# informalsystems/ed25519-consensus

Hardware: AMD Instinct MI355X
Metric: Ed25519 batch-verified signatures/sec (whole node) at 2^20 sigs (higher is better)
Workload: dtype u32/u64 integer (GF(2^255-19), radix 2^29 limbs); 1 GPU; configs[2]: 2^20 votes/GPU from 150 validators, 120-byte msgs; sigs_per_gpu=1048576, validators=150, msg_len=120, inflight=6, keycache=False, prehashed=False, batches_per_launch=1, multi_union_first=False, parallelism=single

## Files before the change

ed25519-consensus_amd/csrc/edc_api.hip:

```cpp
#include <stdlib.h>
#include <string.h>
#include <string>
#include <random>
#include <algorithm>
#include <chrono>
#include <condition_variable>
#include <initializer_list>
#include <mutex>
#include <thread>
#include <unordered_map>
#include <vector>
#include <errno.h>
#include <sys/random.h>
#include <hip/hip_ext.h>
#include "edc.h"
#include "edc_common.h"
#include "edc_launch.h"
#include "vfy_fold.h"
#include "vfy_cached.h"
#include "tmpl.h"
#include "commits.h"
#include "quorum.h"
#include "valset.h"
#include "vhist.h"
// ... 456 lines not shown
    else dens[w] = nf / half;
    total += split ? ns + 2 * nf : (w < P.nwin_short ? ns + nf : nf);
  }
  double target = ctx->bin_entries ? (double)ctx->bin_entries : (total / 1024.0 > 4096.0 ? total / 1024.0 : 4096.0);
  for (;;) {
    for (uint32_t w = 0; w < P.nwin; ++w) P.nsub[w] = (uint8_t)floor_pow2(dens[w] / target);
    plan_layout(P);
    if (P.bins_per_range <= MSM_MAX_BINS) break;
    target *= 2;
  }
  note_plan(ctx, P, target, per_sig, split, few, false);
  return P;
}

static MsmTerms batch_terms(const MsmPlan& P, const Slot& s, uint32_t n, bool split, uint32_t skip = 0) {
  return MsmTerms{n - skip, 0, 0, 0, P.sum_ranges ? P.nranges : 1u, s.scal, nullptr, nullptr, nullptr, split ? 1u : 0u,
                  0u, skip};
}

static bool choose_split(const edc_ctx* ctx) {
  return ctx->kc_m && ctx->bcomb && ctx->key_split == 0 && ctx->last_uncached == 0;
}

static int ensure_n(edc_ctx* ctx, size_t n) {
  CK(grow_group(ctx->cap_n, n, item_cap, sync_of(ctx->st()), [&](size_t cap) {
    return alloc_all(sized(ctx->vtab, verify_single_scratch_words(cap)), sized(ctx->vk, cap * 32), sized(ctx->sig, cap * 64),
                     sized(ctx->zexp, cap * 16), sized(ctx->off, cap + 1), sized(ctx->kbuf, cap * 8), sized(ctx->verdicts, cap));
  }));
  return 0;
}

// ... 132 lines not shown
  x = (x ^ (x >> 30)) * 0xBF58476D1CE4E5B9ull;
  x = (x ^ (x >> 27)) * 0x94D049BB133111EBull;
  return x ^ (x >> 31);
}

static bool choose_per_sig(const edc_ctx* ctx, size_t n) {
  return ctx->key_grouping == 2 || (ctx->key_grouping == 0 && n >= 4096 && ctx->have_key_ratio &&
                                    ctx->last_key_ratio > 0.5 && ctx->ungrouped_run < 7);
}

static uint32_t key_lanes(const edc_ctx* ctx, size_t n, bool per_sig) {
  if (per_sig || !ctx->have_key_ratio) return (uint32_t)n;
  const double m2 = 2.0 * ctx->last_key_ratio * (double)n;
  const size_t lanes = m2 < 4096.0 ? 4096 : (size_t)m2 + 64;
  return (uint32_t)(lanes < n ? lanes : n);
}

static void slot_begin(Slot& s, const uint32_t* kin, uint32_t nmulti, bool timed, bool per_sig, uint32_t n) {
  s.kin = kin;
  s.nmulti = nmulti;
  s.timed = timed;
  s.per_sig = per_sig;
  s.n_batch = n;
}
static size_t batch_entry_room(const MsmPlan& P, size_t n, bool split) {
  return split ? msm_entry_capacity(P, 2 + 3 * n, 0) : msm_entry_capacity(P, n, n + 1);
}
static uint32_t batch_term_count(uint32_t n, bool split) { return split ? 2 + 3 * n : 1 + 2 * n; }

struct KeyTable {
// ... 49 lines not shown
  mark(PH_KEYS);
  const bool clear_counts = with_bin && EDC_RUN(8);
  launch_front(st, s, kt, N, d_vk, clear_counts ? s.msm.counts.get() : nullptr, clear_counts ? P->nbin() : 0u);
  const bool dual = EDC_DUAL_STREAM && s.st2 && !s.timed;
  mark(PH_CHALLENGE);
  if (!d_k && EDC_RUN(2)) launch_challenge(st, N, d_vk, d_sig, in.msg, in.off, s.k);
  if (dual) {
    CK(hipEventRecord(s.ev_keys, st));
    CK(hipStreamWaitEvent(s.st2, s.ev_keys, 0));
    if (EDC_RUN(16))
      launch_decompress(s.st2, N, d_sig, d_vk, s.key_rep, per_sig, s.pts, s.itembad + s.cap_n, s.keybad, s.flags,
                        ctx->kc(), split, key_lanes(ctx, n, per_sig));
    CK(hipEventRecord(s.ev_dec, s.st2));
  }
  mark(PH_COEF);
  if (EDC_RUN(4)) launch_coef(st, N, d_sig, s.kin, d_z, seed, in.z_base, s.key_index, s.scal, s.key_acc, s.u_acc, s.itembad, s.flags,
              per_sig, s.coef_part, split);
  mark(PH_MSM_BIN);
  if (with_bin && EDC_RUN(8))
    launch_msm_bin(st, *P, batch_terms(*P, s, N, split), batch_term_count(N, split), s.msm, s.flags, true);
  if (with_bin && EDC_RUN(256)) launch_msm_sort(st, *P, s.msm);
  mark(PH_DECOMP);
  if (dual) CK(hipStreamWaitEvent(st, s.ev_dec, 0));
  else if (EDC_RUN(16))
    launch_decompress(st, N, d_sig, d_vk, s.key_rep, per_sig, s.pts, s.itembad + s.cap_n, s.keybad, s.flags, ctx->kc(),
                      split, key_lanes(ctx, n, per_sig));
  CK(hipGetLastError());
  return 0;
}

static int enqueue_batch(edc_ctx* ctx, Slot& s, size_t n, const BatchIn& in, bool latency = false) {
  if (n >= (1ull << 28)) { ctx->err = "batch too large for one call (max 2^28 items)"; return EDC_ERR_ARG; }
  int rc = ensure_slot(ctx, s, n);
  if (rc) return rc;
  const bool per_sig = choose_per_sig(ctx, n), split = choose_split(ctx);
// ... 5365 lines not shown
```

ed25519-consensus_amd/csrc/edc_common.h:

```cpp
#pragma once
#include <hip/hip_runtime.h>
#include <stdint.h>
#include "fe25519.h"
#include "ge25519.h"
#include "sc25519.h"
#include "sha512.h"
#include "chacha20.h"
#include "keycache.h"

namespace edc {

constexpr int NIELS_WORDS = 32;
constexpr int EXT_WORDS = 36;

__device__ __forceinline__ fe ld_fe(const uint32_t* p) {
  fe r;
#pragma unroll
  for (int i = 0; i < 9; ++i) r.v[i] = p[i];
  return r;
}
__device__ __forceinline__ void st_fe(uint32_t* p, const fe& a) {
#pragma unroll
  for (int i = 0; i < 9; ++i) p[i] = a.v[i];
}
// ... 40 lines not shown
constexpr int SLICE_BITS = 8;
constexpr int NSLICE = 1 << SLICE_BITS;
constexpr uint32_t MSM_MAX_BINS = 8192;

struct MsmPlan {
  uint32_t nwin, nwin_short;
  uint32_t nranges;
  uint32_t sum_ranges;
  uint32_t bins_per_range;
  uint16_t off[MSM_MAX_WIN];
  uint8_t bits[MSM_MAX_WIN];
  uint8_t nsub[MSM_MAX_WIN];
  uint16_t bin0[MSM_MAX_WIN];
  uint16_t nslice[MSM_MAX_WIN];
  __host__ __device__ uint32_t nbin() const { return nranges * bins_per_range; }
};

struct MsmTerms {
  uint32_t n, rsize, npoint, nx;
  uint32_t nparts;
  const uint32_t* scal;
  const uint32_t* xpt;
  const uint32_t* xrg;
  const uint32_t* xscal;
  uint32_t split;
  uint32_t dyn;
  uint32_t skip;
};

__device__ __forceinline__ int plan_digit(const uint32_t s[8], uint32_t off, uint32_t bits, int& carry,
                                          bool top_unsigned) {
  const uint32_t k = off >> 5, sh = off & 31;
  const uint64_t two = (uint64_t)s[k] | ((uint64_t)(k < 7 ? s[k + 1] : 0u) << 32);
  const uint32_t raw = ((uint32_t)(two >> sh) & ((1u << bits) - 1u)) + (uint32_t)carry;
  if (top_unsigned) { carry = 0; return (int)raw; }
  if (raw >= (1u << (bits - 1))) { carry = 1; return (int)raw - (int)(1u << bits); }
  carry = 0;
  return (int)raw;
}

constexpr int KEY_ACC_LIMBS = 12;

enum { FLAG_BAD = 0, FLAG_NKEYS = 1, FLAG_VERDICT = 2, FLAG_OVF = 3, FLAG_UNCACHED = 4, FLAG_KARG = 5, FLAG_COUNT = 8 };
constexpr int FLAG_ALLOC = 32, FLAG_STAMP0 = 16;
enum { BST_INIT, BST_COEF, BST_COUNT, BST_DECODE, BST_ACCUM, BST_REDUCE, BST_FINAL, BST_END, BST_N };
#ifdef EDC_BATCH_STAMPS
#define BATCH_STAMP(fl, k)                                                                          \
  do {                                                                                              \
    if (blockIdx.x == 0 && threadIdx.x == 0 && (fl))                                                \
      const_cast<int*>(fl)[FLAG_STAMP0 + (k)] = (int)__builtin_amdgcn_s_memrealtime();              \
  } while (0)
#else
#define BATCH_STAMP(fl, k) do { } while (0)
// ... 17 lines not shown
```

ed25519-consensus_amd/csrc/edc_launch.h:

```cpp
#pragma once
#include <hip/hip_runtime.h>
#include <stdint.h>
#include "keycache.h"
#include "edc_common.h"
#include "devbuf.h"

namespace edc {
void launch_challenge(hipStream_t st, uint32_t n, const uint8_t* vk, const uint8_t* sig,
                      const uint8_t* msg, const uint64_t* off, uint32_t* k);
void launch_decompress(hipStream_t st, uint32_t n, const uint8_t* sig, const uint8_t* vk, const uint32_t* key_rep,
                       bool per_sig, uint32_t* pts, uint8_t* itembad, uint8_t* keybad, int* flags,
                       const KeyCacheView& kc, bool split = false, uint32_t klanes = 0);
void launch_decompress_range(hipStream_t st, uint32_t n, uint32_t r0, uint32_t rcnt, uint32_t klanes, const uint8_t* sig,
                             const uint8_t* vk, const uint32_t* key_rep, bool per_sig, uint32_t* pts, uint8_t* itembad,
                             uint8_t* keybad, int* flags, const KeyCacheView& kc, bool split = false);
void launch_keys(hipStream_t st, uint32_t n, const uint8_t* vk, uint32_t* table, uint32_t tmask,
                 const uint32_t salt[2], bool force_overflow, uint32_t* slot_key, uint32_t* key_slot_of_sig,
                 uint32_t* key_rep, uint32_t* key_index, unsigned long long* key_acc, int* flags,
                 uint32_t kcap = 0xFFFFFFFFu);
void launch_keys_range(hipStream_t st, uint32_t n0, uint32_t m, const uint8_t* vk, uint32_t* table, uint32_t tmask,
                       const uint32_t salt[2], bool force_overflow, bool seed_pass, uint32_t* slot_key,
                       uint32_t* key_slot_of_sig, uint32_t* key_rep, uint32_t* key_index, unsigned long long* key_acc,
                       uint32_t* kpts, uint32_t* khi, uint8_t* keybad, int* flags, const KeyCacheView& kc);
void launch_verifier_begin(hipStream_t st, uint32_t n, int* flags, unsigned long long* key_acc,
                           unsigned long long* u_acc, uint8_t* d_out, uint32_t* counts, uint32_t nbin);
void launch_verifier_place_keys(hipStream_t st, uint32_t n, const uint8_t* vk, const uint32_t* kpts, const uint32_t* khi,
                                uint32_t* pts, uint8_t* keybad, int* flags, const KeyCacheView& kc, bool split);
void launch_z_range(hipStream_t st, const uint32_t seed[8], uint32_t a, uint32_t cnt, uint32_t* scal);
void launch_coef(hipStream_t st, uint32_t n, const uint8_t* sig, const uint32_t* k, const uint8_t* zexp,
                 const uint32_t seed[8], uint64_t zbase, const uint32_t* key_index, uint32_t* scal,
                 unsigned long long* key_acc, unsigned long long* u_acc, uint8_t* itembad, int* flags,
                 bool per_sig, uint32_t* coef_part, bool split = false);
void launch_coef_range(hipStream_t st, uint32_t n, uint32_t item0, uint32_t cnt, const uint8_t* sig, const uint32_t* k,
                       const uint8_t* zexp, const uint32_t seed[8], uint64_t zbase, const uint32_t* key_index,
                       uint32_t* scal, unsigned long long* key_acc, unsigned long long* u_acc, uint8_t* itembad,
                       int* flags, bool per_sig, uint32_t* coef_part, bool split = false);
void launch_coef_finish(hipStream_t st, uint32_t n, unsigned long long* key_acc, unsigned long long* u_acc,
                        uint32_t* scal, int* flags, bool per_sig, uint32_t* coef_part, bool split = false);
size_t coef_part_words(size_t cap_n);
void launch_range_coef(hipStream_t st, uint32_t n, uint32_t rsize, uint32_t nranges, uint32_t m, bool per_sig,
                       const uint8_t* sig, const uint32_t* k, const uint8_t* zexp, const uint32_t seed[8],
                       uint64_t zbase, const uint32_t* key_index, uint32_t* scal, unsigned long long* key_acc,
                       unsigned long long* u_acc, int* flags, uint32_t* xpt, uint32_t* xrg, uint32_t* xscal);
void launch_multi_coef(hipStream_t st, uint32_t n, uint32_t nr, uint32_t kstride, bool per_sig, const uint8_t* sig,
                       const uint32_t* k, const uint32_t seed[8], uint64_t zbase, const uint32_t* key_index,
                       uint32_t* scal, unsigned long long* key_acc, unsigned long long* u_acc, uint8_t* itembad,
                       int* flags, uint32_t* xpt, uint32_t* xrg, uint32_t* xscal);
// ... 114 lines not shown
void launch_header_bind(hipStream_t st, const HeaderSrc& src, const HeaderBind& rules, const uint8_t* roots, uint8_t* bad,
                        uint32_t* n_bad);
hipError_t msm_init_device();
struct MsmWs {
  uint32_t cap_bins = 0, cap_ranges = 0;
  size_t cap_entries = 0;
  devbuf::DevBuf<uint32_t> counts, offsets, cursor;
  devbuf::DevBuf<uint2> entries;
  devbuf::DevBuf<uint32_t> sorted;
  devbuf::DevBuf<uint32_t> slice_W, slice_T, win;
  devbuf::DevBuf<uint32_t> buckets;
  devbuf::DevBuf<uint32_t> heads;
  devbuf::DevBuf<uint32_t> bucket_end;
};
void launch_msm_bin(hipStream_t st, const MsmPlan& P, const MsmTerms& T, uint32_t max_terms, MsmWs& ws, const int* flags,
                    bool counts_zeroed = false);
void launch_msm_sort(hipStream_t st, const MsmPlan& P, MsmWs& ws);
void launch_msm_bucket(hipStream_t st, const MsmPlan& P, MsmWs& ws, const uint32_t* pts, int probe_skip = 0,
                       hipEvent_t acc_begin = nullptr, hipEvent_t acc_end = nullptr, bool latency = false,
                       int* stamp_flags = nullptr);
size_t msm_bucket_words(uint32_t nbin);
void launch_msm_tail(hipStream_t st, const MsmPlan& P, MsmWs& ws, int* flags, int want_compress, uint8_t* out,
                     uint8_t* hout = nullptr, const uint32_t* extra = nullptr);
void launch_point_accum(hipStream_t st, uint32_t* run, const uint8_t* blk);
void launch_msm_range_tail(hipStream_t st, const MsmPlan& P, MsmWs& ws, uint8_t* rverdict);
void launch_msm_multi_tail(hipStream_t st, const MsmPlan& P, MsmWs& ws, const int* flags, const uint8_t* rbad,
                           int want_compress, uint8_t* out, uint8_t* hout);
void launch_combine_records(hipStream_t st, uint32_t g, const uint8_t* recs, uint32_t stride, uint8_t* out);
void launch_combine(hipStream_t st, uint32_t g, const uint8_t* partials, int bad, int want_compress,
                    uint8_t* out);
void launch_copy_block(hipStream_t st, const uint8_t* src, uint8_t* dst);
// ... 21 lines not shown
```

ed25519-consensus_amd/csrc/edc_msm.hip:

```cpp
#include "edc_common.h"
#include "edc_launch.h"
#include "ge_quad.h"
#include "ge_row.h"

namespace edc {


__device__ __forceinline__ MsmTerms resolve_terms(MsmTerms T, const int* flags) {
  if (T.dyn & 1u) {
    const bool per_sig = (T.dyn & 2u) || flags[FLAG_OVF];
    const uint32_t nr = T.nx, m = per_sig ? 0u : (uint32_t)flags[FLAG_NKEYS];
    T.npoint = per_sig ? 2 * T.n : T.n;
    T.nx = nr * m + nr;
  }
  return T;
}

__device__ __forceinline__ uint32_t terms_count(const MsmTerms& T, const int* flags) {
  if (T.rsize) return T.npoint + T.nx;
  const uint32_t m = (uint32_t)flags[FLAG_NKEYS];
  return T.split ? msm_num_points_split(T.n, m) : msm_num_points(T.n, m);
}

__device__ __forceinline__ void term_get(const MsmTerms& T, uint32_t t, uint32_t& pt, uint32_t& rg, bool& shrt,
                                         uint32_t s[8]) {
  const uint32_t* src;
  if (!T.rsize) {
    pt = t ? t + T.skip : 0u;
    rg = T.nparts > 1 ? t % T.nparts : 0;
    shrt = T.split || (t >= 1 && t <= T.n);
    src = T.scal + (size_t)pt * 8;
  } else if (t < T.npoint) {
    pt = 1 + T.skip + t;
    rg = (t < T.n ? t : t - T.n) / T.rsize;
    shrt = t < T.n;
    src = T.scal + (size_t)pt * 8;
  } else {
    const uint32_t q = t - T.npoint;
    pt = T.xpt[q];
    rg = T.xrg[q];
    shrt = false;
    src = T.xscal + (size_t)q * 8;
  }
  const uint4* q4 = reinterpret_cast<const uint4*>(src);
  const uint4 a = q4[0], b = shrt ? make_uint4(0u, 0u, 0u, 0u) : q4[1];
  s[0] = a.x; s[1] = a.y; s[2] = a.z; s[3] = a.w; s[4] = b.x; s[5] = b.y; s[6] = b.z; s[7] = b.w;
}

template <typename F>
__device__ __forceinline__ void term_digits(const MsmPlan& P, uint32_t t, bool shrt, uint32_t rg, const uint32_t s[8],
                                            F&& f) {
  const uint32_t nw = shrt ? P.nwin_short : P.nwin;
  const uint32_t rbase = rg * P.bins_per_range;
  int carry = 0;
  for (uint32_t w = 0; w < nw; ++w) {
    const int d = plan_digit(s, P.off[w], P.bits[w], carry, w + 1 == nw);
    if (d) {
      const uint32_t b = (uint32_t)(d < 0 ? -d : d) - 1;
      const uint32_t ns = P.nsub[w];
      f(rbase + P.bin0[w] + (b >> SLICE_BITS) * ns + (t & (ns - 1)), b & (NSLICE - 1), d < 0);
    }
  }
}

__global__ void __launch_bounds__(256) k_msm_count(MsmPlan P, MsmTerms T, uint32_t per_block,
                                                   uint32_t* __restrict__ counts, const int* __restrict__ flags) {
  extern __shared__ uint32_t hist[];
  BATCH_STAMP(flags, BST_COUNT);
  const uint32_t nbin = P.nbin();
  for (uint32_t b = threadIdx.x; b < nbin; b += blockDim.x) hist[b] = 0;
  __syncthreads();
  T = resolve_terms(T, flags);
  const uint32_t cnt = terms_count(T, flags);
  const uint32_t t0 = blockIdx.x * per_block;
  for (uint32_t u = threadIdx.x; u < per_block; u += blockDim.x) {
    const uint32_t t = t0 + u;
    if (t >= cnt) break;
    uint32_t pt, rg, s[8];
    bool shrt;
    term_get(T, t, pt, rg, shrt, s);
    term_digits(P, t, shrt, rg, s, [&](uint32_t bin, uint32_t, bool) { atomicAdd(&hist[bin], 1u); });
  }
  __syncthreads();
  for (uint32_t b = threadIdx.x; b < nbin; b += blockDim.x)
    if (hist[b]) atomicAdd(&counts[b], hist[b]);
}

__global__ void __launch_bounds__(1024) k_msm_scan(uint32_t nbin, const uint32_t* __restrict__ counts,
                                                   uint32_t* __restrict__ offsets,
                                                   uint32_t* __restrict__ cursor) {
  __shared__ uint32_t part[1024];
  const uint32_t t = threadIdx.x;
  const uint32_t per = (nbin + 1023) / 1024;
  const uint32_t b0 = t * per, b1 = min(nbin, b0 + per);
  uint32_t s = 0;
  for (uint32_t b = b0; b < b1; ++b) s += counts[b];
  part[t] = s;
  __syncthreads();
  for (int d = 1; d < 1024; d <<= 1) {
    uint32_t v = t >= (uint32_t)d ? part[t - d] : 0;
    __syncthreads();
    part[t] += v;
    __syncthreads();
  }
  uint32_t run = part[t] - s;
  for (uint32_t b = b0; b < b1; ++b) {
    offsets[b] = run;
    cursor[b] = run;
    run += counts[b];
  }
}

struct ScatterBlocks {
  uint32_t grid_a, per_a, a0, a_end, per_b, b_base;
};
template <typename F>
__device__ __forceinline__ void scatter_terms(const ScatterBlocks& S, uint32_t cnt, F&& f) {
  if (blockIdx.x < S.grid_a) {
    const uint32_t t0 = S.a0 + blockIdx.x * S.per_a, lim = min(cnt, S.a_end);
    for (uint32_t u = threadIdx.x; u < S.per_a; u += blockDim.x) {
      if (t0 + u >= lim) break;
      f(t0 + u);
    }
  } else {
    const uint32_t v0 = (blockIdx.x - S.grid_a) * S.per_b;
// ... 775 lines not shown
__global__ void k_copy_block(const uint4* __restrict__ src, uint4* __restrict__ dst) {
  if (threadIdx.x < 16) dst[threadIdx.x] = src[threadIdx.x];
}

static inline uint32_t cdiv(uint64_t a, uint32_t b) { return (uint32_t)((a + b - 1) / b); }
static constexpr size_t kScatterLdsMax = 160 * 1024 - 256;
#ifndef EDC_SCATTER_STAGE
#define EDC_SCATTER_STAGE 16384
#endif
static uint32_t g_scatter_stage_max = EDC_SCATTER_STAGE;
extern "C" int edc_debug_set_scatter_stage(uint32_t max_entries) {
  g_scatter_stage_max = max_entries > 16384 ? 16384u : max_entries;
  return 0;
}

void launch_msm_bin(hipStream_t st, const MsmPlan& P, const MsmTerms& T, uint32_t max_terms, MsmWs& ws, const int* flags,
                    bool counts_zeroed) {
  const uint32_t nbin = P.nbin();
  if (!counts_zeroed) (void)hipMemsetAsync(ws.counts, 0, nbin * sizeof(uint32_t), st);
  uint32_t per = max_terms / 256;
  per = per < 256 ? 256 : (per > 4096 ? 4096 : (per + 255) / 256 * 256);
  const size_t lds_max = kScatterLdsMax, bins_bytes = (3 * (size_t)nbin + 1) * sizeof(uint32_t);
  uint32_t stage_cap = bins_bytes + 2048 * sizeof(uint2) <= lds_max
                           ? (uint32_t)std::min<size_t>(g_scatter_stage_max, (lds_max - bins_bytes) / sizeof(uint2) / 256 * 256)
                           : 0u;
  const uint32_t grid = cdiv(max_terms ? max_terms : 1, per);
  ScatterBlocks SB{grid, per, 0u, 0xFFFFFFFFu, per, 0u};
  uint32_t sgrid = grid;
  if (stage_cap) {
    const auto fit = [&](uint32_t digits) { return stage_cap / std::max(1u, digits) / 256 * 256; };
    const uint32_t fa = fit(P.nwin_short), fb = fit(P.nwin);
    if (!T.rsize && !T.split && P.nwin > P.nwin_short && fa >= 256 && fb >= 256) {
// ... 1 lines not shown
      SB.per_b = std::min(per, fb);
      SB.a0 = 1;
      SB.a_end = 1 + T.n;
      SB.b_base = T.n;
      SB.grid_a = cdiv(T.n ? T.n : 1, SB.per_a);
      sgrid = SB.grid_a + cdiv(max_terms > T.n ? max_terms - T.n : 1, SB.per_b);
    } else if (fa >= 256 && per > fa) {
      SB.per_a = SB.per_b = fa;
      SB.grid_a = sgrid = cdiv(max_terms ? max_terms : 1, fa);
    }
  }
#ifndef EDC_COUNT_SPLIT
#define EDC_COUNT_SPLIT 4
#endif
  const uint32_t cper = std::max(256u, per / EDC_COUNT_SPLIT);
  hipLaunchKernelGGL(k_msm_count, dim3(cdiv(max_terms ? max_terms : 1, cper)), dim3(256), nbin * sizeof(uint32_t), st, P, T,
                     cper, ws.counts.get(), flags);
  hipLaunchKernelGGL(k_msm_scan, dim3(1), dim3(1024), 0, st, nbin, ws.counts.get(), ws.offsets.get(), ws.cursor.get());
#ifdef EDC_PROBE_EXTRA_SCANS
  for (int r = 0; r < EDC_PROBE_EXTRA_SCANS; ++r)
    hipLaunchKernelGGL(k_msm_scan, dim3(1), dim3(1024), 0, st, nbin, ws.counts.get(), ws.offsets.get(), ws.cursor.get());
#endif
  hipLaunchKernelGGL(k_msm_scatter, dim3(sgrid), dim3(SCATTER_THREADS), bins_bytes + (size_t)stage_cap * sizeof(uint2), st, P, T,
                     SB, ws.cursor.get(), ws.entries.get(), flags, stage_cap);
}

hipError_t msm_init_device() {
  return hipFuncSetAttribute(reinterpret_cast<const void*>(&k_msm_scatter), hipFuncAttributeMaxDynamicSharedMemorySize,
                             (int)kScatterLdsMax);
}

static const size_t kReduceLds = (size_t)NSLICE * EXT_WORDS * sizeof(uint32_t);

// ... 110 lines not shown
```

ed25519-consensus_amd/csrc/edc_prep.hip:

```cpp
#include "edc_common.h"
#include "edc_launch.h"
#include "ge_quad.h"

namespace edc {

constexpr int SHA_CLASSES = 16;
constexpr int SHA_THREADS = 256;
#ifndef EDC_SHA_OCC
#define EDC_SHA_OCC 4
#endif
#ifndef EDC_SHA_STAGED
#define EDC_SHA_STAGED 1
#endif

constexpr int SHA_WIN_CHUNKS = 9;
__device__ __attribute__((aligned(16))) uint32_t g_sha_zero[4];

__device__ __forceinline__ void sha_dma16(const void* gsrc, uint32_t* lds_row) {
  __builtin_amdgcn_global_load_lds((const __attribute__((address_space(1))) void*)gsrc,
                                   (__attribute__((address_space(3))) void*)lds_row, 16, 0, 0);
}

__device__ __forceinline__ uint32_t* sha_col(uint32_t* wbuf, uint32_t lane, uint32_t x) {
  return wbuf + (x >> 2) * 256 + lane * 4 + (x & 3);
// ... 439 lines not shown
#pragma unroll
  for (int i = 0; i < PL; ++i) r[i] = 0;
#pragma unroll
  for (int i = 0; i < 4; ++i) {
    uint64_t c = 0;
#pragma unroll
    for (int j = 0; j < 8; ++j) {
      uint64_t t = (uint64_t)z[i] * s[j] + r[i + j] + c;
      r[i + j] = (uint32_t)t;
      c = t >> 32;
    }
    r[i + 8] = (uint32_t)c;
  }
}

__global__ void __launch_bounds__(256) k_coef(uint32_t n, const uint8_t* __restrict__ sig,
                                              const uint32_t* __restrict__ kscal,
                                              const uint8_t* __restrict__ zexp, seed8 seed,
                                              uint64_t zbase, const uint32_t* __restrict__ key_index,
                                              uint32_t* __restrict__ scal,
                                              unsigned long long* __restrict__ key_acc,
                                              unsigned long long* __restrict__ u_acc,
                                              uint8_t* __restrict__ itembad,
                                              int* __restrict__ flags, int per_sig_host, uint32_t rsize, uint32_t m,
                                              uint32_t* __restrict__ coef_part, int split, uint32_t item0,
                                              uint32_t iend) {
  __shared__ uint32_t tag[COEF_SLOTS];
  __shared__ unsigned long long acc[COEF_SLOTS][PL];
  __shared__ unsigned long long red[4][PL];
  BATCH_STAMP(flags, BST_COEF);
  const bool per_sig = per_sig_host || flags[FLAG_OVF];
  for (int s = threadIdx.x; s < COEF_SLOTS; s += blockDim.x) {
    tag[s] = 0xFFFFFFFFu;
#pragma unroll
    for (int j = 0; j < PL; ++j) acc[s][j] = 0;
  }
  __syncthreads();
  unsigned long long ua[PL];
#pragma unroll
  for (int j = 0; j < PL; ++j) ua[j] = 0;
  bool bad = false, karg = false;
  const uint32_t wg = item0 / COEF_CHUNK + blockIdx.x, nwg = (n + COEF_CHUNK - 1) / COEF_CHUNK;
  const uint32_t base = wg * COEF_CHUNK;
  const uint32_t pair0 = rsize ? (base / rsize) * m : 0u;
  for (int grp = 0; grp < COEF_SIGS_PER_THREAD / 4; ++grp) {
    const uint32_t i0 = base + 4 * (threadIdx.x + 256 * grp);
    if (i0 >= iend) break;
    uint32_t blk[16];
    const bool aligned = ((zbase + i0) & 3) == 0;
    if (!zexp && aligned) chacha20_block(seed.w, (zbase + i0) >> 2, blk);
#pragma unroll
    for (int q = 0; q < 4; ++q) {
      const uint32_t i = i0 + q;
      if (i >= iend) break;
      uint32_t z[4];
      if (zexp) {
        const uint4 zz = *reinterpret_cast<const uint4*>(zexp + (size_t)i * 16);
        z[0] = zz.x; z[1] = zz.y; z[2] = zz.z; z[3] = zz.w;
      } else if (aligned) {
#pragma unroll
        for (int j = 0; j < 4; ++j) z[j] = blk[4 * q + j];
      } else {
        uint32_t b2[16];
        chacha20_block(seed.w, (zbase + i) >> 2, b2);
        const int o = (int)((zbase + i) & 3);
// ... 5 lines not shown
      const uint4* kp = reinterpret_cast<const uint4*>(kscal + (size_t)i * 8);
      uint4 k0 = kp[0], k1 = kp[1];
      kw[0] = k0.x; kw[1] = k0.y; kw[2] = k0.z; kw[3] = k0.w; kw[4] = k1.x; kw[5] = k1.y; kw[6] = k1.z; kw[7] = k1.w;
      const bool s_bad = !sc_is_canonical(sw);
      bad |= s_bad;
      karg |= !sc_is_canonical(kw);
      if (itembad) itembad[i] = s_bad ? ITEM_BAD_S : 0;
      uint32_t u[PL], v[PL];
      mul_128x256(z, sw, u);
      mul_128x256(z, kw, v);
#pragma unroll
      for (int j = 0; j < PL; ++j) ua[j] += u[j];
      uint4* sp = reinterpret_cast<uint4*>(scal + (size_t)(1 + i) * 8);
      sp[0] = make_uint4(z[0], z[1], z[2], z[3]);
      sp[1] = make_uint4(0, 0, 0, 0);
      if (per_sig) {
        uint32_t x[16];
#pragma unroll
        for (int j = 0; j < 16; ++j) x[j] = j < PL ? v[j] : 0u;
        const sc a = sc_reduce_wide(x);
        uint4* ap = reinterpret_cast<uint4*>(scal + (size_t)(1 + n + i) * 8);
        ap[0] = make_uint4(a.v[0], a.v[1], a.v[2], a.v[3]);
        if (split) {
          ap[1] = make_uint4(0, 0, 0, 0);
          uint4* hp = reinterpret_cast<uint4*>(scal + (size_t)split_hi_point(n, n, i) * 8);
          hp[0] = make_uint4(a.v[4], a.v[5], a.v[6], a.v[7]);
          hp[1] = make_uint4(0, 0, 0, 0);
        } else {
          ap[1] = make_uint4(a.v[4], a.v[5], a.v[6], a.v[7]);
        }
        continue;
      }
      const uint32_t key = pair0 + key_index[i];
      const uint32_t slot = key & (COEF_SLOTS - 1);
      const uint32_t prev = atomicCAS(&tag[slot], 0xFFFFFFFFu, key);
      if (prev == 0xFFFFFFFFu || prev == key) {
#pragma unroll
        for (int j = 0; j < PL; ++j) atomicAdd(&acc[slot][j], (unsigned long long)v[j]);
      } else {
#pragma unroll
        for (int j = 0; j < PL; ++j) atomicAdd(&key_acc[(size_t)key * PL + j], (unsigned long long)v[j]);
      }
    }
  }
  if (bad) atomicOr(&flags[FLAG_BAD], 1);
  if (karg) atomicOr(&flags[FLAG_KARG], 1);
#pragma unroll
  for (int j = 0; j < PL; ++j) {
    unsigned long long x = ua[j];
#pragma unroll
    for (int d = 32; d >= 1; d >>= 1) x += __shfl_down(x, d, 64);
    ua[j] = x;
  }
  const int lane = threadIdx.x & 63, wv = threadIdx.x >> 6;
  if (lane == 0) {
#pragma unroll
    for (int j = 0; j < PL; ++j) red[wv][j] = ua[j];
  }
  __syncthreads();
  if (threadIdx.x < PL) {
    unsigned long long x = red[0][threadIdx.x] + red[1][threadIdx.x] + red[2][threadIdx.x] + red[3][threadIdx.x];
    atomicAdd(&u_acc[(rsize ? (size_t)(base / rsize) * PL : 0) + threadIdx.x], x);
  }
  if (coef_part) {
    uint32_t* ptag = coef_part + (size_t)wg * COEF_SLOTS;
    unsigned long long* psum = coef_part_sums(coef_part, nwg) + (size_t)wg * COEF_SLOTS * PL;
    for (int s = threadIdx.x; s < COEF_SLOTS; s += blockDim.x) {
      ptag[s] = tag[s];
      if (tag[s] != 0xFFFFFFFFu) {
#pragma unroll
        for (int j = 0; j < PL; ++j) psum[(size_t)s * PL + j] = acc[s][j];
      }
    }
    return;
  }
  for (int s = threadIdx.x; s < COEF_SLOTS; s += blockDim.x) {
    const uint32_t key = tag[s];
// ... 232 lines not shown
  for (uint32_t j = i; j < nbin; j += stride) counts[j] = 0;
}

void launch_init_batch(hipStream_t st, int* flags, int nkeys, unsigned long long* u_acc, uint8_t* d_out, uint32_t* table,
                       uint32_t T, uint32_t* counts, uint32_t nbin) {
  const uint32_t work = T > nbin ? T : nbin;
  uint32_t grid = cdiv(work > 256 ? work : 256, 256);
  if (grid > 4096) grid = 4096;
  hipLaunchKernelGGL(k_init_batch, dim3(grid), dim3(256), 0, st, flags, nkeys, u_acc, reinterpret_cast<uint32_t*>(d_out),
                     table, T, counts, nbin);
}

void launch_coef(hipStream_t st, uint32_t n, const uint8_t* sig, const uint32_t* k, const uint8_t* zexp,
                 const uint32_t seed[8], uint64_t zbase, const uint32_t* key_index, uint32_t* scal,
                 unsigned long long* key_acc, unsigned long long* u_acc, uint8_t* itembad, int* flags,
                 bool per_sig, uint32_t* coef_part, bool split) {
  seed8 s;
  for (int j = 0; j < 8; ++j) s.w[j] = seed[j];
  if (n) {
    const uint32_t nwg = cdiv(n, COEF_CHUNK);
    uint32_t* part = per_sig ? nullptr : coef_part;
    hipLaunchKernelGGL(k_coef, dim3(nwg), dim3(256), 0, st, n, sig, k, zexp, s, zbase, key_index, scal, key_acc,
                       u_acc, itembad, flags, per_sig ? 1 : 0, 0u, 0u, part, split ? 1 : 0, 0u, n);
  }
  launch_coef_finish(st, n, key_acc, u_acc, scal, flags, per_sig, coef_part, split);
}
void launch_coef_range(hipStream_t st, uint32_t n, uint32_t item0, uint32_t cnt, const uint8_t* sig, const uint32_t* k,
                       const uint8_t* zexp, const uint32_t seed[8], uint64_t zbase, const uint32_t* key_index,
                       uint32_t* scal, unsigned long long* key_acc, unsigned long long* u_acc, uint8_t* itembad,
                       int* flags, bool per_sig, uint32_t* coef_part, bool split) {
  seed8 s;
  for (int j = 0; j < 8; ++j) s.w[j] = seed[j];
  if (cnt)
    hipLaunchKernelGGL(k_coef, dim3(cdiv(cnt, COEF_CHUNK)), dim3(256), 0, st, n, sig, k, zexp, s, zbase, key_index,
                       scal, key_acc, u_acc, itembad, flags, per_sig ? 1 : 0, 0u, 0u, per_sig ? nullptr : coef_part,
                       split ? 1 : 0, item0, item0 + cnt);
}
void launch_coef_finish(hipStream_t st, uint32_t n, unsigned long long* key_acc, unsigned long long* u_acc,
                        uint32_t* scal, int* flags, bool per_sig, uint32_t* coef_part, bool split) {
  if (n && !per_sig)
    hipLaunchKernelGGL(k_coef_merge, dim3(COEF_SLOTS), dim3(256), 0, st, cdiv(n, COEF_CHUNK), coef_part, key_acc);
  hipLaunchKernelGGL(k_key_final, dim3(grid_cap(cdiv(n > 0 ? n : 1, 256), 1024)), dim3(256), 0, st, n, key_acc,
                     u_acc, scal, flags, per_sig ? 1 : 0, split ? 1 : 0);
}
__global__ void __launch_bounds__(256) k_z_range(seed8 seed, uint32_t a, uint32_t cnt, uint32_t* __restrict__ scal) {
  const uint32_t b0 = a >> 2, nblk = ((a + cnt + 3) >> 2) - b0;
  const uint32_t g = blockIdx.x * blockDim.x + threadIdx.x;
  if (g >= nblk) return;
  uint32_t blk[16];
  chacha20_block(seed.w, (uint64_t)(b0 + g), blk);
#pragma unroll
// ... 16 lines not shown
size_t coef_part_words(size_t cap_n) {
  const size_t nwg = (cap_n + COEF_CHUNK - 1) / COEF_CHUNK;
  return ((nwg * COEF_SLOTS + 1) & ~(size_t)1) + nwg * COEF_SLOTS * PL * 2;
}

void launch_range_coef(hipStream_t st, uint32_t n, uint32_t rsize, uint32_t nranges, uint32_t m, bool per_sig,
                       const uint8_t* sig, const uint32_t* k, const uint8_t* zexp, const uint32_t seed[8],
                       uint64_t zbase, const uint32_t* key_index, uint32_t* scal, unsigned long long* key_acc,
                       unsigned long long* u_acc, int* flags, uint32_t* xpt, uint32_t* xrg, uint32_t* xscal) {
  seed8 s;
  for (int j = 0; j < 8; ++j) s.w[j] = seed[j];
  const uint32_t mm = per_sig ? 0u : m;
  (void)hipMemsetAsync(key_acc, 0, (size_t)nranges * mm * PL * sizeof(unsigned long long), st);
  (void)hipMemsetAsync(u_acc, 0, (size_t)nranges * PL * sizeof(unsigned long long), st);
  if (n)
    hipLaunchKernelGGL(k_coef, dim3(cdiv(n, COEF_CHUNK)), dim3(256), 0, st, n, sig, k, zexp, s, zbase,
                       key_index, scal, key_acc, u_acc, (uint8_t*)nullptr, flags, per_sig ? 1 : 0, rsize, mm,
                       (uint32_t*)nullptr, 0, 0u, n);
  hipLaunchKernelGGL(k_range_terms, dim3(grid_cap(cdiv((uint64_t)nranges * (mm + 1), 256), 1024)), dim3(256), 0, st,
                     n, nranges, mm, key_acc, u_acc, xpt, xrg, xscal);
}
void launch_multi_coef(hipStream_t st, uint32_t n, uint32_t nr, uint32_t kstride, bool per_sig, const uint8_t* sig,
                       const uint32_t* k, const uint32_t seed[8], uint64_t zbase, const uint32_t* key_index,
                       uint32_t* scal, unsigned long long* key_acc, unsigned long long* u_acc, uint8_t* itembad,
                       int* flags, uint32_t* xpt, uint32_t* xrg, uint32_t* xscal) {
  seed8 s;
  for (int j = 0; j < 8; ++j) s.w[j] = seed[j];
  if (!per_sig) (void)hipMemsetAsync(key_acc, 0, (size_t)nr * kstride * PL * sizeof(unsigned long long), st);
  (void)hipMemsetAsync(u_acc, 0, (size_t)nr * PL * sizeof(unsigned long long), st);
  if (n)
    hipLaunchKernelGGL(k_coef, dim3(cdiv(n, COEF_CHUNK)), dim3(256), 0, st, n, sig, k, (const uint8_t*)nullptr, s, zbase,
                       key_index, scal, key_acc, u_acc, itembad, flags, per_sig ? 1 : 0, n / nr, kstride,
                       (uint32_t*)nullptr, 0, 0u, n);
  hipLaunchKernelGGL(k_multi_terms, dim3(grid_cap(cdiv((uint64_t)nr * (per_sig ? 1 : kstride + 1), 256), 1024)),
                     dim3(256), 0, st, n, nr, kstride, key_acc, u_acc, flags, per_sig ? 1 : 0, xpt, xrg, xscal);
}
void launch_range_prebad(hipStream_t st, uint32_t n, uint32_t rsize, const uint8_t* itembad, const uint8_t* itembad_r,
                         const uint8_t* keybad,
                         const uint32_t* key_index, bool per_sig, uint8_t* rbad, const int* flags) {
  if (n)
    hipLaunchKernelGGL(k_range_prebad, dim3(cdiv(n, 256)), dim3(256), 0, st, n, rsize, itembad, itembad_r, keybad,
                       key_index, per_sig ? 1 : 0, flags, rbad);
}
__global__ void __launch_bounds__(256) k_expand_keys(uint32_t n, const uint32_t* __restrict__ key_idx,
                                                     const uint32_t* __restrict__ reg,
                                                     const uint32_t* __restrict__ keys, uint32_t* __restrict__ vk_out) {
  const uint32_t i = blockIdx.x * blockDim.x + threadIdx.x;
  if (i >= n) return;
// ... 52 lines not shown
```

Measured before the change: 704.0 million sigs/s.

## Count MSM bin histogram for R-terms inside coef kernel; fuse small count with scan

```diff
diff --git a/ed25519-consensus_amd/csrc/edc_api.hip b/ed25519-consensus_amd/csrc/edc_api.hip
--- a/ed25519-consensus_amd/csrc/edc_api.hip
+++ b/ed25519-consensus_amd/csrc/edc_api.hip
@@ -494,7 +494,7 @@
 }
 
 static MsmTerms batch_terms(const MsmPlan& P, const Slot& s, uint32_t n, bool split, uint32_t skip = 0) {
-  return MsmTerms{n - skip, 0, 0, 0, P.sum_ranges ? P.nranges : 1u, s.scal, nullptr, nullptr, nullptr, split ? 1u : 0u,
+  return MsmTerms{n - skip, 0, 0, 0, P.parts(), s.scal, nullptr, nullptr, nullptr, split ? 1u : 0u,
                   0u, skip};
 }
 
@@ -657,6 +657,12 @@
   const double m2 = 2.0 * ctx->last_key_ratio * (double)n;
   const size_t lanes = m2 < 4096.0 ? 4096 : (size_t)m2 + 64;
   return (uint32_t)(lanes < n ? lanes : n);
+}
+
+static uint32_t front_terms(const edc_ctx* ctx, size_t n, bool split) {
+  const double m2 = !ctx->have_key_ratio ? (double)n : 2.0 * ctx->last_key_ratio * (double)n;
+  const size_t keys = m2 < (double)n ? (size_t)m2 : n;
+  return (uint32_t)((split ? 2 : 1) * (1 + keys));
 }
 
 static void slot_begin(Slot& s, const uint32_t* kin, uint32_t nmulti, bool timed, bool per_sig, uint32_t n) {
@@ -736,11 +742,13 @@
     CK(hipEventRecord(s.ev_dec, s.st2));
   }
   mark(PH_COEF);
+  const bool count_at_source = clear_counts && N && !per_sig && EDC_RUN(4);
   if (EDC_RUN(4)) launch_coef(st, N, d_sig, s.kin, d_z, seed, in.z_base, s.key_index, s.scal, s.key_acc, s.u_acc, s.itembad, s.flags,
-              per_sig, s.coef_part, split);
+              per_sig, s.coef_part, split, count_at_source ? P : nullptr, count_at_source ? s.msm.counts.get() : nullptr);
   mark(PH_MSM_BIN);
   if (with_bin && EDC_RUN(8))
-    launch_msm_bin(st, *P, batch_terms(*P, s, N, split), batch_term_count(N, split), s.msm, s.flags, true);
+    launch_msm_bin(st, *P, batch_terms(*P, s, N, split), batch_term_count(N, split), s.msm, s.flags, true,
+                   count_at_source ? front_terms(ctx, n, split) : 0u);
   if (with_bin && EDC_RUN(256)) launch_msm_sort(st, *P, s.msm);
   mark(PH_DECOMP);
   if (dual) CK(hipStreamWaitEvent(st, s.ev_dec, 0));
diff --git a/ed25519-consensus_amd/csrc/edc_common.h b/ed25519-consensus_amd/csrc/edc_common.h
--- a/ed25519-consensus_amd/csrc/edc_common.h
+++ b/ed25519-consensus_amd/csrc/edc_common.h
@@ -78,6 +78,7 @@
   uint16_t bin0[MSM_MAX_WIN];
   uint16_t nslice[MSM_MAX_WIN];
   __host__ __device__ uint32_t nbin() const { return nranges * bins_per_range; }
+  __host__ __device__ uint32_t parts() const { return sum_ranges ? nranges : 1u; }
 };
 
 struct MsmTerms {
@@ -101,6 +102,32 @@
   if (raw >= (1u << (bits - 1))) { carry = 1; return (int)raw - (int)(1u << bits); }
   carry = 0;
   return (int)raw;
+}
+
+template <typename F>
+__device__ __forceinline__ void term_digits(const MsmPlan& P, uint32_t t, bool shrt, uint32_t rg, const uint32_t s[8],
+                                            F&& f) {
+  const uint32_t nw = shrt ? P.nwin_short : P.nwin;
+  const uint32_t rbase = rg * P.bins_per_range;
+  int carry = 0;
+  for (uint32_t w = 0; w < nw; ++w) {
+    const int d = plan_digit(s, P.off[w], P.bits[w], carry, w + 1 == nw);
+    if (d) {
+      const uint32_t b = (uint32_t)(d < 0 ? -d : d) - 1;
+      const uint32_t ns = P.nsub[w];
+      f(rbase + P.bin0[w] + (b >> SLICE_BITS) * ns + (t & (ns - 1)), b & (NSLICE - 1), d < 0);
+    }
+  }
+}
+
+__device__ __forceinline__ uint32_t batch_term_part(uint32_t nparts, uint32_t t) {
+  return nparts > 1 ? t % nparts : 0u;
+}
+
+template <typename F>
+__device__ __forceinline__ void r_term_digits(const MsmPlan& P, uint32_t i, const uint32_t z[4], F&& f) {
+  const uint32_t s[8] = {z[0], z[1], z[2], z[3], 0u, 0u, 0u, 0u};
+  term_digits(P, 1 + i, true, batch_term_part(P.parts(), 1 + i), s, f);
 }
 
 constexpr int KEY_ACC_LIMBS = 12;
diff --git a/ed25519-consensus_amd/csrc/edc_launch.h b/ed25519-consensus_amd/csrc/edc_launch.h
--- a/ed25519-consensus_amd/csrc/edc_launch.h
+++ b/ed25519-consensus_amd/csrc/edc_launch.h
@@ -30,7 +30,8 @@
 void launch_coef(hipStream_t st, uint32_t n, const uint8_t* sig, const uint32_t* k, const uint8_t* zexp,
                  const uint32_t seed[8], uint64_t zbase, const uint32_t* key_index, uint32_t* scal,
                  unsigned long long* key_acc, unsigned long long* u_acc, uint8_t* itembad, int* flags,
-                 bool per_sig, uint32_t* coef_part, bool split = false);
+                 bool per_sig, uint32_t* coef_part, bool split = false, const MsmPlan* bin_plan = nullptr,
+                 uint32_t* bin_counts = nullptr);
 void launch_coef_range(hipStream_t st, uint32_t n, uint32_t item0, uint32_t cnt, const uint8_t* sig, const uint32_t* k,
                        const uint8_t* zexp, const uint32_t seed[8], uint64_t zbase, const uint32_t* key_index,
                        uint32_t* scal, unsigned long long* key_acc, unsigned long long* u_acc, uint8_t* itembad,
@@ -175,7 +176,7 @@
   devbuf::DevBuf<uint32_t> bucket_end;
 };
 void launch_msm_bin(hipStream_t st, const MsmPlan& P, const MsmTerms& T, uint32_t max_terms, MsmWs& ws, const int* flags,
-                    bool counts_zeroed = false);
+                    bool counts_zeroed = false, uint32_t front_terms = 0);
 void launch_msm_sort(hipStream_t st, const MsmPlan& P, MsmWs& ws);
 void launch_msm_bucket(hipStream_t st, const MsmPlan& P, MsmWs& ws, const uint32_t* pts, int probe_skip = 0,
                        hipEvent_t acc_begin = nullptr, hipEvent_t acc_end = nullptr, bool latency = false,
diff --git a/ed25519-consensus_amd/csrc/edc_msm.hip b/ed25519-consensus_amd/csrc/edc_msm.hip
--- a/ed25519-consensus_amd/csrc/edc_msm.hip
+++ b/ed25519-consensus_amd/csrc/edc_msm.hip
@@ -27,7 +27,7 @@
   const uint32_t* src;
   if (!T.rsize) {
     pt = t ? t + T.skip : 0u;
-    rg = T.nparts > 1 ? t % T.nparts : 0;
+    rg = batch_term_part(T.nparts, t);
     shrt = T.split || (t >= 1 && t <= T.n);
     src = T.scal + (size_t)pt * 8;
   } else if (t < T.npoint) {
@@ -47,54 +47,25 @@
   s[0] = a.x; s[1] = a.y; s[2] = a.z; s[3] = a.w; s[4] = b.x; s[5] = b.y; s[6] = b.z; s[7] = b.w;
 }
 
-template <typename F>
-__device__ __forceinline__ void term_digits(const MsmPlan& P, uint32_t t, bool shrt, uint32_t rg, const uint32_t s[8],
-                                            F&& f) {
-  const uint32_t nw = shrt ? P.nwin_short : P.nwin;
-  const uint32_t rbase = rg * P.bins_per_range;
-  int carry = 0;
-  for (uint32_t w = 0; w < nw; ++w) {
-    const int d = plan_digit(s, P.off[w], P.bits[w], carry, w + 1 == nw);
-    if (d) {
-      const uint32_t b = (uint32_t)(d < 0 ? -d : d) - 1;
-      const uint32_t ns = P.nsub[w];
-      f(rbase + P.bin0[w] + (b >> SLICE_BITS) * ns + (t & (ns - 1)), b & (NSLICE - 1), d < 0);
-    }
-  }
-}
-
-__global__ void __launch_bounds__(256) k_msm_count(MsmPlan P, MsmTerms T, uint32_t per_block,
-                                                   uint32_t* __restrict__ counts, const int* __restrict__ flags) {
-  extern __shared__ uint32_t hist[];
-  BATCH_STAMP(flags, BST_COUNT);
-  const uint32_t nbin = P.nbin();
-  for (uint32_t b = threadIdx.x; b < nbin; b += blockDim.x) hist[b] = 0;
-  __syncthreads();
-  T = resolve_terms(T, flags);
-  const uint32_t cnt = terms_count(T, flags);
-  const uint32_t t0 = blockIdx.x * per_block;
-  for (uint32_t u = threadIdx.x; u < per_block; u += blockDim.x) {
-    const uint32_t t = t0 + u;
-    if (t >= cnt) break;
-    uint32_t pt, rg, s[8];
-    bool shrt;
-    term_get(T, t, pt, rg, shrt, s);
-    term_digits(P, t, shrt, rg, s, [&](uint32_t bin, uint32_t, bool) { atomicAdd(&hist[bin], 1u); });
-  }
-  __syncthreads();
-  for (uint32_t b = threadIdx.x; b < nbin; b += blockDim.x)
-    if (hist[b]) atomicAdd(&counts[b], hist[b]);
-}
-
-__global__ void __launch_bounds__(1024) k_msm_scan(uint32_t nbin, const uint32_t* __restrict__ counts,
-                                                   uint32_t* __restrict__ offsets,
-                                                   uint32_t* __restrict__ cursor) {
-  __shared__ uint32_t part[1024];
+__device__ __forceinline__ uint32_t count_terms(const MsmTerms& T, uint32_t cnt, int skip_r) {
+  return skip_r ? cnt - T.n : cnt;
+}
+__device__ __forceinline__ uint32_t count_term(const MsmTerms& T, uint32_t u, int skip_r) {
+  return skip_r && u ? T.n + u : u;
+}
+
+__device__ __forceinline__ void scan_bins(uint32_t nbin, uint32_t* __restrict__ counts, const uint32_t* add,
+                                          uint32_t* __restrict__ offsets, uint32_t* __restrict__ cursor,
+                                          uint32_t* part) {
   const uint32_t t = threadIdx.x;
   const uint32_t per = (nbin + 1023) / 1024;
-  const uint32_t b0 = t * per, b1 = min(nbin, b0 + per);
+  const uint32_t b0 = min(nbin, t * per), b1 = min(nbin, b0 + per);
   uint32_t s = 0;
-  for (uint32_t b = b0; b < b1; ++b) s += counts[b];
+  for (uint32_t b = b0; b < b1; ++b) {
+    uint32_t c = counts[b];
+    if (add && add[b]) { c += add[b]; counts[b] = c; }
+    s += c;
+  }
   part[t] = s;
   __syncthreads();
   for (int d = 1; d < 1024; d <<= 1) {
@@ -109,6 +80,44 @@
     cursor[b] = run;
     run += counts[b];
   }
+}
+
+template <bool FRONT>
+__global__ void __launch_bounds__(FRONT ? 1024 : 256) k_msm_count(MsmPlan P, MsmTerms T, uint32_t per_block, int skip_r,
+                                                                  uint32_t* __restrict__ counts,
+                                                                  uint32_t* __restrict__ offsets,
+                                                                  uint32_t* __restrict__ cursor,
+                                                                  const int* __restrict__ flags) {
+  extern __shared__ uint32_t hist[];
+  __shared__ uint32_t part[FRONT ? 1024 : 1];
+  BATCH_STAMP(flags, BST_COUNT);
+  const uint32_t nbin = P.nbin();
+  for (uint32_t b = threadIdx.x; b < nbin; b += blockDim.x) hist[b] = 0;
+  __syncthreads();
+  T = resolve_terms(T, flags);
+  const uint32_t cnt = count_terms(T, terms_count(T, flags), skip_r);
+  const uint32_t u0 = FRONT ? 0u : blockIdx.x * per_block, u1 = FRONT ? cnt : min(cnt, u0 + per_block);
+  for (uint32_t u = u0 + threadIdx.x; u < u1; u += blockDim.x) {
+    const uint32_t t = count_term(T, u, skip_r);
+    uint32_t pt, rg, s[8];
+    bool shrt;
+    term_get(T, t, pt, rg, shrt, s);
+    term_digits(P, t, shrt, rg, s, [&](uint32_t bin, uint32_t, bool) { atomicAdd(&hist[bin], 1u); });
+  }
+  __syncthreads();
+  if (FRONT) {
+    scan_bins(nbin, counts, hist, offsets, cursor, part);
+    return;
+  }
+  for (uint32_t b = threadIdx.x; b < nbin; b += blockDim.x)
+    if (hist[b]) atomicAdd(&counts[b], hist[b]);
+}
+
+__global__ void __launch_bounds__(1024) k_msm_scan(uint32_t nbin, uint32_t* __restrict__ counts,
+                                                   uint32_t* __restrict__ offsets,
+                                                   uint32_t* __restrict__ cursor) {
+  __shared__ uint32_t part[1024];
+  scan_bins(nbin, counts, nullptr, offsets, cursor, part);
 }
 
 struct ScatterBlocks {
@@ -914,8 +923,10 @@
   return 0;
 }
 
+static constexpr uint32_t kFrontFuseMax = 8192;
+
 void launch_msm_bin(hipStream_t st, const MsmPlan& P, const MsmTerms& T, uint32_t max_terms, MsmWs& ws, const int* flags,
-                    bool counts_zeroed) {
+                    bool counts_zeroed, uint32_t front_terms) {
   const uint32_t nbin = P.nbin();
   if (!counts_zeroed) (void)hipMemsetAsync(ws.counts, 0, nbin * sizeof(uint32_t), st);
   uint32_t per = max_terms / 256;
@@ -947,9 +958,16 @@
 #define EDC_COUNT_SPLIT 4
 #endif
   const uint32_t cper = std::max(256u, per / EDC_COUNT_SPLIT);
-  hipLaunchKernelGGL(k_msm_count, dim3(cdiv(max_terms ? max_terms : 1, cper)), dim3(256), nbin * sizeof(uint32_t), st, P, T,
-                     cper, ws.counts.get(), flags);
-  hipLaunchKernelGGL(k_msm_scan, dim3(1), dim3(1024), 0, st, nbin, ws.counts.get(), ws.offsets.get(), ws.cursor.get());
+  const int skip_r = front_terms ? 1 : 0;
+  if (skip_r && front_terms <= kFrontFuseMax) {
+    hipLaunchKernelGGL(k_msm_count<true>, dim3(1), dim3(1024), nbin * sizeof(uint32_t), st, P, T, 0u, 1, ws.counts.get(),
+                       ws.offsets.get(), ws.cursor.get(), flags);
+  } else {
+    const uint32_t cterms = skip_r ? max_terms - std::min(max_terms, T.n) : max_terms;
+    hipLaunchKernelGGL(k_msm_count<false>, dim3(cdiv(cterms ? cterms : 1, cper)), dim3(256), nbin * sizeof(uint32_t), st, P,
+                       T, cper, skip_r, ws.counts.get(), (uint32_t*)nullptr, (uint32_t*)nullptr, flags);
+    hipLaunchKernelGGL(k_msm_scan, dim3(1), dim3(1024), 0, st, nbin, ws.counts.get(), ws.offsets.get(), ws.cursor.get());
+  }
 #ifdef EDC_PROBE_EXTRA_SCANS
   for (int r = 0; r < EDC_PROBE_EXTRA_SCANS; ++r)
     hipLaunchKernelGGL(k_msm_scan, dim3(1), dim3(1024), 0, st, nbin, ws.counts.get(), ws.offsets.get(), ws.cursor.get());
diff --git a/ed25519-consensus_amd/csrc/edc_prep.hip b/ed25519-consensus_amd/csrc/edc_prep.hip
--- a/ed25519-consensus_amd/csrc/edc_prep.hip
+++ b/ed25519-consensus_amd/csrc/edc_prep.hip
@@ -477,7 +477,17 @@
   }
 }
 
-__global__ void __launch_bounds__(256) k_coef(uint32_t n, const uint8_t* __restrict__ sig,
+struct CoefBin {
+  MsmPlan P;
+  uint32_t* counts;
+};
+#ifdef EDC_COEF_WAVES
+#define COEF_WAVES __attribute__((amdgpu_waves_per_eu(EDC_COEF_WAVES, EDC_COEF_WAVES)))
+#else
+#define COEF_WAVES
+#endif
+template <bool BIN>
+__global__ void __launch_bounds__(256) COEF_WAVES k_coef(uint32_t n, const uint8_t* __restrict__ sig,
                                               const uint32_t* __restrict__ kscal,
                                               const uint8_t* __restrict__ zexp, seed8 seed,
                                               uint64_t zbase, const uint32_t* __restrict__ key_index,
@@ -487,7 +497,8 @@
                                               uint8_t* __restrict__ itembad,
                                               int* __restrict__ flags, int per_sig_host, uint32_t rsize, uint32_t m,
                                               uint32_t* __restrict__ coef_part, int split, uint32_t item0,
-                                              uint32_t iend) {
+                                              uint32_t iend, CoefBin bin) {
+  extern __shared__ uint32_t hist[];
   __shared__ uint32_t tag[COEF_SLOTS];
   __shared__ unsigned long long acc[COEF_SLOTS][PL];
   __shared__ unsigned long long red[4][PL];
@@ -498,6 +509,8 @@
 #pragma unroll
     for (int j = 0; j < PL; ++j) acc[s][j] = 0;
   }
+  if (BIN)
+    for (uint32_t b = threadIdx.x; b < bin.P.nbin(); b += blockDim.x) hist[b] = 0;
   __syncthreads();
   unsigned long long ua[PL];
 #pragma unroll
@@ -512,6 +525,7 @@
     uint32_t blk[16];
     const bool aligned = ((zbase + i0) & 3) == 0;
     if (!zexp && aligned) chacha20_block(seed.w, (zbase + i0) >> 2, blk);
+    uint32_t zq[4][4];
 #pragma unroll
     for (int q = 0; q < 4; ++q) {
       const uint32_t i = i0 + q;
@@ -547,6 +561,10 @@
       uint4* sp = reinterpret_cast<uint4*>(scal + (size_t)(1 + i) * 8);
       sp[0] = make_uint4(z[0], z[1], z[2], z[3]);
       sp[1] = make_uint4(0, 0, 0, 0);
+      if (BIN) {
+#pragma unroll
+        for (int j = 0; j < 4; ++j) zq[q][j] = z[j];
+      }
       if (per_sig) {
         uint32_t x[16];
 #pragma unroll
@@ -575,6 +593,12 @@
         for (int j = 0; j < PL; ++j) atomicAdd(&key_acc[(size_t)key * PL + j], (unsigned long long)v[j]);
       }
     }
+    if (BIN) {
+#pragma unroll
+      for (int q = 0; q < 4; ++q)
+        if (i0 + q < iend)
+          r_term_digits(bin.P, i0 + q, zq[q], [&](uint32_t b, uint32_t, bool) { atomicAdd(&hist[b], 1u); });
+    }
   }
   if (bad) atomicOr(&flags[FLAG_BAD], 1);
   if (karg) atomicOr(&flags[FLAG_KARG], 1);
@@ -594,6 +618,10 @@
   if (threadIdx.x < PL) {
     unsigned long long x = red[0][threadIdx.x] + red[1][threadIdx.x] + red[2][threadIdx.x] + red[3][threadIdx.x];
     atomicAdd(&u_acc[(rsize ? (size_t)(base / rsize) * PL : 0) + threadIdx.x], x);
+  }
+  if (BIN) {
+    for (uint32_t b = threadIdx.x; b < bin.P.nbin(); b += blockDim.x)
+      if (hist[b]) atomicAdd(&bin.counts[b], hist[b]);
   }
   if (coef_part) {
     uint32_t* ptag = coef_part + (size_t)wg * COEF_SLOTS;
@@ -856,14 +884,19 @@
 void launch_coef(hipStream_t st, uint32_t n, const uint8_t* sig, const uint32_t* k, const uint8_t* zexp,
                  const uint32_t seed[8], uint64_t zbase, const uint32_t* key_index, uint32_t* scal,
                  unsigned long long* key_acc, unsigned long long* u_acc, uint8_t* itembad, int* flags,
-                 bool per_sig, uint32_t* coef_part, bool split) {
+                 bool per_sig, uint32_t* coef_part, bool split, const MsmPlan* bin_plan, uint32_t* bin_counts) {
   seed8 s;
   for (int j = 0; j < 8; ++j) s.w[j] = seed[j];
   if (n) {
     const uint32_t nwg = cdiv(n, COEF_CHUNK);
     uint32_t* part = per_sig ? nullptr : coef_part;
-    hipLaunchKernelGGL(k_coef, dim3(nwg), dim3(256), 0, st, n, sig, k, zexp, s, zbase, key_index, scal, key_acc,
-                       u_acc, itembad, flags, per_sig ? 1 : 0, 0u, 0u, part, split ? 1 : 0, 0u, n);
+    if (bin_plan && bin_counts)
+      hipLaunchKernelGGL(k_coef<true>, dim3(nwg), dim3(256), bin_plan->nbin() * sizeof(uint32_t), st, n, sig, k, zexp, s,
+                         zbase, key_index, scal, key_acc, u_acc, itembad, flags, per_sig ? 1 : 0, 0u, 0u, part,
+                         split ? 1 : 0, 0u, n, CoefBin{*bin_plan, bin_counts});
+    else
+      hipLaunchKernelGGL(k_coef<false>, dim3(nwg), dim3(256), 0, st, n, sig, k, zexp, s, zbase, key_index, scal, key_acc,
+                         u_acc, itembad, flags, per_sig ? 1 : 0, 0u, 0u, part, split ? 1 : 0, 0u, n, CoefBin{});
   }
   launch_coef_finish(st, n, key_acc, u_acc, scal, flags, per_sig, coef_part, split);
 }
@@ -874,9 +907,9 @@
   seed8 s;
   for (int j = 0; j < 8; ++j) s.w[j] = seed[j];
   if (cnt)
-    hipLaunchKernelGGL(k_coef, dim3(cdiv(cnt, COEF_CHUNK)), dim3(256), 0, st, n, sig, k, zexp, s, zbase, key_index,
+    hipLaunchKernelGGL(k_coef<false>, dim3(cdiv(cnt, COEF_CHUNK)), dim3(256), 0, st, n, sig, k, zexp, s, zbase, key_index,
                        scal, key_acc, u_acc, itembad, flags, per_sig ? 1 : 0, 0u, 0u, per_sig ? nullptr : coef_part,
-                       split ? 1 : 0, item0, item0 + cnt);
+                       split ? 1 : 0, item0, item0 + cnt, CoefBin{});
 }
 void launch_coef_finish(hipStream_t st, uint32_t n, unsigned long long* key_acc, unsigned long long* u_acc,
                         uint32_t* scal, int* flags, bool per_sig, uint32_t* coef_part, bool split) {
@@ -923,9 +956,9 @@
   (void)hipMemsetAsync(key_acc, 0, (size_t)nranges * mm * PL * sizeof(unsigned long long), st);
   (void)hipMemsetAsync(u_acc, 0, (size_t)nranges * PL * sizeof(unsigned long long), st);
   if (n)
-    hipLaunchKernelGGL(k_coef, dim3(cdiv(n, COEF_CHUNK)), dim3(256), 0, st, n, sig, k, zexp, s, zbase,
+    hipLaunchKernelGGL(k_coef<false>, dim3(cdiv(n, COEF_CHUNK)), dim3(256), 0, st, n, sig, k, zexp, s, zbase,
                        key_index, scal, key_acc, u_acc, (uint8_t*)nullptr, flags, per_sig ? 1 : 0, rsize, mm,
-                       (uint32_t*)nullptr, 0, 0u, n);
+                       (uint32_t*)nullptr, 0, 0u, n, CoefBin{});
   hipLaunchKernelGGL(k_range_terms, dim3(grid_cap(cdiv((uint64_t)nranges * (mm + 1), 256), 1024)), dim3(256), 0, st,
                      n, nranges, mm, key_acc, u_acc, xpt, xrg, xscal);
 }
@@ -938,9 +971,9 @@
   if (!per_sig) (void)hipMemsetAsync(key_acc, 0, (size_t)nr * kstride * PL * sizeof(unsigned long long), st);
   (void)hipMemsetAsync(u_acc, 0, (size_t)nr * PL * sizeof(unsigned long long), st);
   if (n)
-    hipLaunchKernelGGL(k_coef, dim3(cdiv(n, COEF_CHUNK)), dim3(256), 0, st, n, sig, k, (const uint8_t*)nullptr, s, zbase,
+    hipLaunchKernelGGL(k_coef<false>, dim3(cdiv(n, COEF_CHUNK)), dim3(256), 0, st, n, sig, k, (const uint8_t*)nullptr, s, zbase,
                        key_index, scal, key_acc, u_acc, itembad, flags, per_sig ? 1 : 0, n / nr, kstride,
-                       (uint32_t*)nullptr, 0, 0u, n);
+                       (uint32_t*)nullptr, 0, 0u, n, CoefBin{});
   hipLaunchKernelGGL(k_multi_terms, dim3(grid_cap(cdiv((uint64_t)nr * (per_sig ? 1 : kstride + 1), 256), 1024)),
                      dim3(256), 0, st, n, nr, kstride, key_acc, u_acc, flags, per_sig ? 1 : 0, xpt, xrg, xscal);
 }
```

Result: no change. 702.2 million sigs/s (-0.3%).
